# martinResearch/PySparseLP

Hardware: AMD Instinct MI355X
Metric: admm_iterations_per_sec (higher is better)
Workload: dtype f64

## Files before the change

### pysparselp_amd/csrc/slp_tall.h

```cpp
#pragma once
#include "slp_common.h"

namespace slp {

constexpr int kTallC = 4096;
constexpr int kTallT = 1024;
constexpr int kTallSlots = 8;
constexpr int kTallDepth = 4;
constexpr int kTallDictMax = 2048;
constexpr int kTallBuckets = 6;
constexpr int kTallIdBits = 11, kTallColBits = 12, kTallRowBits = 14;
constexpr int kTallCellShift = kTallIdBits + kTallColBits + kTallRowBits;
static_assert(kTallBuckets * 32 == 3 * kWave, "k_tall_build scans the (count, bank class) buckets three per lane of one wave");
static_assert(kTallRmax < (1 << kTallRowBits) && kTallC == (1 << kTallColBits) && kTallDictMax == (1 << kTallIdBits), "tall geometry");
static_assert((kTallRmax + 1) * 8 + kTallDictMax * 8 + 2 * kTallC * 8 <= 160 * 1024, "tall cells: LDS budget");

constexpr unsigned int kPktNewCell = 0x80000000u;
constexpr unsigned int kNoTile = 0x7fffffffu;
constexpr unsigned int kOob = 0xffffff00u;

struct TallPkt {
    unsigned int off;
    unsigned int xsrc;
    unsigned int c[4];
    unsigned int strip;
    unsigned int pad;
};
static_assert(sizeof(TallPkt) == 32, "packet header");

__host__ __device__ inline unsigned long long tall_value_key(unsigned long long bits) {
    return (bits >> 63) ? ~bits : (bits | 0x8000000000000000ull);
}

}
```

### pysparselp_amd/csrc/slp_tall_spmv.hip

```cpp
#include <cmath>
#include <cstdlib>
#include <cstring>
#include <vector>

#include "slp_common.h"
#include "slp_kernels.h"
#include "slp_tall.h"

namespace slp {


template <bool DICT>
struct TallRegs {
    unsigned int lo[kTallSlots];
    unsigned int hi[DICT ? 2 : 1];
    double val[DICT ? 1 : kTallSlots];
    double x[4];
};

template <bool DICT, bool ACC, bool POW = false, int C = kTallC>
__global__ __launch_bounds__(kTallT) void k_tall_spmv(int nseg, const TallWg *__restrict__ wgs, const double *__restrict__ dict_arg,
                                                      const double *__restrict__ x, double *__restrict__ out, double pw) {
    constexpr int kDepth = DICT ? kTallDepth : 2;
    __shared__ double acc[kTallRmax + 1];
    __shared__ double dv[kTallDictMax];
    static_assert(C == 4096 || C == 2048 || C == 1024, "tall cells: strip width");
    __shared__ double xt[2][C];
    constexpr int kPieces = C / 2048 ? C / 2048 : 1;
    const int p = threadIdx.x;
    const bool tile_lane = C >= 2048 || p < C / 2;
    const unsigned int wbase = (unsigned int)__builtin_amdgcn_readfirstlane(p & ~(kWave - 1));
    const int v = blockIdx.x;
    int cur = 0;
    TallWg wg = wgs[v];
    for (int r = p; r <= wg.nrows; r += kTallT) acc[r] = (ACC && r > 0) ? out[wg.row0 + r - 1] : 0.0;
  for (int seg = 0; seg < nseg; ++seg) {
    if (seg > 0) wg = wgs[(i64)seg * gridDim.x + v];
    if (DICT) {
        const double *__restrict__ dsrc = dict_arg ? dict_arg : wg.dict;
        for (int q = p; q < wg.D; q += kTallT) dv[q] = dsrc[q];
    }
    typedef const unsigned int __attribute__((address_space(1))) *gptr_t;
    const gptr_t hd = (gptr_t)(unsigned long long)wg.dir + (p & 7);
    const int npk = (int)wg.npk - 2 * kTallDepth;
    const __amdgpu_buffer_rsrc_t rs_x =
        __builtin_amdgcn_make_buffer_rsrc(const_cast<double *>(x + wg.x0), 0, (int)(wg.ncol * 8), 0x00020000);

    auto slot_pay = [&](unsigned int so, unsigned int width) {
        return __builtin_amdgcn_make_buffer_rsrc(const_cast<unsigned int *>(wg.pay) + so, 0, (int)(width * 4u), 0x00020000);
    };
    auto slot_val = [&](unsigned int so, unsigned int width) {
        return __builtin_amdgcn_make_buffer_rsrc(const_cast<double *>(DICT ? x : wg.val) + so, 0, (int)(width * 8u), 0x00020000);
    };

    TallRegs<DICT> regs[kDepth];
    unsigned int hw[2 * kDepth];

    auto widths = [&](unsigned int h, unsigned int *c) {
#pragma unroll
        for (int i = 0; i < 4; ++i) {
            const unsigned int v = (unsigned int)__builtin_amdgcn_readlane((int)h, 2 + i);
            c[2 * i] = v & 0xffffu;
            c[2 * i + 1] = v >> 16;
        }
    };

    auto load_tile = [&](TallRegs<DICT> &g, const unsigned int xo) {
#pragma unroll
        for (int i = 0; i < kPieces; ++i) {
            const auto v = __builtin_amdgcn_raw_buffer_load_b128(rs_x, xo + (unsigned int)i * (unsigned int)(C * 4), 0, 0);
            g.x[2 * i] = __hiloint2double((int)v[1], (int)v[0]);
            g.x[2 * i + 1] = __hiloint2double((int)v[3], (int)v[2]);
        }
    };

    auto issue = [&](TallRegs<DICT> &g, unsigned int h) {
        const unsigned int off = (unsigned int)__builtin_amdgcn_readlane((int)h, 0);
        const unsigned int xs = (unsigned int)__builtin_amdgcn_readlane((int)h, 1) & 0x7fffffffu;
        unsigned int c[kTallSlots];
        widths(h, c);
        unsigned int so = off;
        const unsigned int mine = (unsigned int)p * 4u;
#pragma unroll
        for (int k = 0; k < kTallSlots; ++k) {
            g.lo[k] = __builtin_amdgcn_raw_buffer_load_b32(slot_pay(so, c[k]), mine, 0, 2);
            if (!DICT) {
                const auto v = __builtin_amdgcn_raw_buffer_load_b64(slot_val(so, c[k]), 2u * mine, 0, 2);
                g.val[k] = __hiloint2double((int)v[1], (int)v[0]);
            }
            so += c[k];
        }
        if (DICT) {
            g.hi[0] = __builtin_amdgcn_raw_buffer_load_b32(slot_pay(so, c[0]), mine, 0, 2);
            so += c[0];
            g.hi[DICT ? 1 : 0] = __builtin_amdgcn_raw_buffer_load_b32(slot_pay(so, c[4]), mine, 0, 2);
        }
        const unsigned int xo = (xs == kNoTile || !tile_lane) ? kOob : (xs + 2u * (unsigned int)p) * 8u;
        load_tile(g, xo);
    };

    auto issue_part = [&](TallRegs<DICT> &g, unsigned int h, const int part) {
        const unsigned int off = (unsigned int)__builtin_amdgcn_readlane((int)h, 0);
        unsigned int c[kTallSlots];
        widths(h, c);
        const unsigned int mine = (unsigned int)p * 4u;
        unsigned int so = off;
        if (part == 1) so += c[0] + c[1] + c[2] + c[3];
        if (part == 0 || wbase < c[4]) {
#pragma unroll
            for (int k = 4 * part; k < 4 * part + 4; ++k) {
                g.lo[k] = __builtin_amdgcn_raw_buffer_load_b32(slot_pay(so, c[k]), mine, 0, 2);
                if (!DICT) {
                    const auto v = __builtin_amdgcn_raw_buffer_load_b64(slot_val(so, c[k]), 2u * mine, 0, 2);
                    g.val[DICT ? 0 : k] = __hiloint2double((int)v[1], (int)v[0]);
                }
                so += c[k];
            }
            if (DICT) {
                if (part == 0) so += c[4] + c[5] + c[6] + c[7];
                else so += c[0];
                g.hi[DICT ? part : 0] = __builtin_amdgcn_raw_buffer_load_b32(slot_pay(so, c[4 * part]), mine, 0, 2);
            }
        }
        if (part == 1) {
            const unsigned int xs = (unsigned int)__builtin_amdgcn_readlane((int)h, 1) & 0x7fffffffu;
            const unsigned int xo = (xs == kNoTile || !tile_lane) ? kOob : (xs + 2u * (unsigned int)p) * 8u;
            load_tile(g, xo);
        }
    };

    auto consume = [&](TallRegs<DICT> &g, unsigned int h, unsigned int hnext, auto &&between) {
        const unsigned int xw = (unsigned int)__builtin_amdgcn_readlane((int)h, 1);
        const unsigned int c4 = (unsigned int)__builtin_amdgcn_readlane((int)h, 4) & 0xffffu;
        if (xw & kPktNewCell) {
            asm volatile("s_waitcnt lgkmcnt(0)\n\ts_barrier" ::: "memory");
            cur ^= 1;
        }
        auto stage_tile = [&]() {
            if ((xw & 0x7fffffffu) != kNoTile) {
                double *dst = &xt[cur ^ 1][2 * p];
                if (tile_lane) *reinterpret_cast<double2 *>(dst) = make_double2(g.x[0], g.x[1]);
                if (kPieces == 2) *reinterpret_cast<double2 *>(dst + C / 2) = make_double2(g.x[2], g.x[3]);
            }
        };
        stage_tile();
        const double *__restrict__ tile = xt[cur];
        auto group = [&](const int k0) {
            unsigned int w[4], hb[4], row[4];
            double ar[4], pr[4], t[4];
#pragma unroll
            for (int k = 0; k < 4; ++k) {
                w[k] = g.lo[k0 + k];
                if (DICT) {
                    hb[k] = (g.hi[DICT ? (k0 >> 2) : 0] >> (8 * k)) & 0xffu;
                    row[k] = (w[k] >> 23) | (hb[k] << 9);
                } else {
                    hb[k] = 0;
                    row[k] = w[k] >> kTallColBits;
                }
            }
#pragma unroll
            for (int k = 0; k < 4; ++k) ar[k] = acc[row[k]];
#pragma unroll
            for (int k = 0; k < 4; ++k) {
                pr[k] = DICT ? dv[w[k] & ((1u << kTallIdBits) - 1)] * tile[(w[k] >> kTallIdBits) & (kTallC - 1)]
                             : (POW ? abs_pow(g.val[DICT ? 0 : k0 + k], pw) * 1.0 : g.val[DICT ? 0 : k0 + k]) * tile[w[k] & (kTallC - 1)];
            }
            t[0] = ar[0] + pr[0];
#pragma unroll
            for (int k = 1; k < 4; ++k) t[k] = ((row[k] == row[k - 1]) ? t[k - 1] : ar[k]) + pr[k];
#pragma unroll
            for (int k = 0; k < 4; ++k) acc[row[k]] = t[k];
        };
        group(0);
        between();
        if (wbase < c4) group(4);
    };

#pragma unroll
    for (int u = 0; u < 2 * kDepth; ++u) hw[u] = hd[(i64)u * 8];
#pragma unroll
    for (int u = 0; u < kDepth; ++u) issue(regs[u], hw[u]);
    __syncthreads();
    for (int jj = 0; jj < npk; jj += 2 * kDepth) {
#pragma unroll
        for (int u = 0; u < 2 * kDepth; ++u) {
            consume(regs[u % kDepth], hw[u], hw[(u + kDepth) % (2 * kDepth)], [&]() { issue_part(regs[u % kDepth], hw[(u + kDepth) % (2 * kDepth)], 0); });
            issue_part(regs[u % kDepth], hw[(u + kDepth) % (2 * kDepth)], 1);
            hw[u] = hd[(i64)(jj + u + 2 * kDepth) * 8];
        }
    }
    __syncthreads();
  }
    for (int r = p; r < wg.nrows; r += kTallT) out[wg.row0 + r] = acc[r + 1];
}


__global__ void k_tall_combine(i64 nrow, int S, const double *__restrict__ part, double *__restrict__ out, int accum) {
    for (i64 r = (i64)blockIdx.x * blockDim.x + threadIdx.x; r < nrow; r += (i64)gridDim.x * blockDim.x) {
        double a = accum ? out[r] + part[r] : part[r];
        for (int s = 1; s < S; ++s) a += part[(i64)s * nrow + r];
        out[r] = a;
    }
}

template <bool DICT, bool ACC, bool POW>
static void tall_launch(int C, unsigned grid, int nseg, const TallWg *wgs, const double *dict, const double *x, double *out, double pw) {
    switch (C) {
    case 4096: hipLaunchKernelGGL((k_tall_spmv<DICT, ACC, POW, 4096>), dim3(grid), dim3(kTallT), 0, ctx().stream, nseg, wgs, dict, x, out, pw); break;
    case 2048: hipLaunchKernelGGL((k_tall_spmv<DICT, ACC, POW, 2048>), dim3(grid), dim3(kTallT), 0, ctx().stream, nseg, wgs, dict, x, out, pw); break;
    case 1024: hipLaunchKernelGGL((k_tall_spmv<DICT, ACC, POW, 1024>), dim3(grid), dim3(kTallT), 0, ctx().stream, nseg, wgs, dict, x, out, pw); break;
    default: SLP_REQUIRE(false, "tall cells: strip width");
    }
}

void tall_spmv(const StripJds &f, const double *x, double *out, int accum) {
    double *dst = f.S > 1 ? f.part.p : out;
    const unsigned grid = (unsigned)(f.B * f.S);
    const bool acc = accum && f.S == 1;
    const double *none = nullptr;
    if (f.D > 0) { if (acc) tall_launch<true, true, false>((int)f.C, grid, 1, f.tall_wg.p, f.dict, x, dst, 0.0); else tall_launch<true, false, false>((int)f.C, grid, 1, f.tall_wg.p, f.dict, x, dst, 0.0); }
    else { if (acc) tall_launch<false, true, false>((int)f.C, grid, 1, f.tall_wg.p, none, x, dst, 0.0); else tall_launch<false, false, false>((int)f.C, grid, 1, f.tall_wg.p, none, x, dst, 0.0); }
    if (f.S > 1)
        hipLaunchKernelGGL(k_tall_combine, dim3(grid_for(f.nrow, kBlock)), dim3(kBlock), 0, ctx().stream, f.nrow, f.S, f.part.p, out, accum);
    SLP_HIP(hipGetLastError());
}

void tall_spmv_fused(const StripJds &f, const double *x, double *out) {
    const int nseg = f.parts_cols ? (int)f.parts.size() : 1;
    const unsigned grid = (unsigned)(f.tall_wg.n / (size_t)nseg);
    if (f.D > 0) tall_launch<true, false, false>((int)f.C, grid, nseg, f.tall_wg.p, nullptr, x, out, 0.0);
    else tall_launch<false, false, false>((int)f.C, grid, nseg, f.tall_wg.p, nullptr, x, out, 0.0);
    SLP_HIP(hipGetLastError());
}

bool tall_fuse(StripJds &f) {
    f.tall_wg.release();
    const char *e = getenv("SLP_TALL_FUSE");
    if (e && e[0] == '0') return false;
    if (f.parts.empty()) return false;
    const StripJds &f0 = *f.parts[0];
    for (const StripJds *g : f.parts)
        if (!g->ok || !g->tall || g->S != 1 || g->C != f0.C || (g->D > 0) != (f0.D > 0) || (f.parts_cols && (g->B != f0.B || g->tall_R != f0.tall_R || g->nrow != f0.nrow)))
            return false;
    std::vector<TallWg> all;
    for (size_t k = 0; k < f.parts.size(); ++k) {
        const StripJds &g = *f.parts[k];
        std::vector<TallWg> wg((size_t)g.B);
        SLP_HIP(hipMemcpy(wg.data(), g.tall_wg.p, wg.size() * sizeof(TallWg), hipMemcpyDeviceToHost));
        for (TallWg &w : wg) {
            w.dict = g.dict;
            if (f.parts_cols) w.x0 = f.part_off[k];
            else w.row0 += f.part_off[k];
            all.push_back(w);
        }
    }
    f.tall_wg.upload(all.data(), all.size());
    f.C = f0.C;
    return true;
}

void tall_spmv_pow(const StripJds &f, double pw, const double *x, double *out, int accum) {
    SLP_REQUIRE(f.ok && f.tall && f.D == 0, "tall_spmv_pow: not a tall-cell copy with fp64 entries");
    double *dst = f.S > 1 ? f.part.p : out;
    const unsigned grid = (unsigned)(f.B * f.S);
    if (accum && f.S == 1) tall_launch<false, true, true>((int)f.C, grid, 1, f.tall_wg.p, nullptr, x, dst, pw);
    else tall_launch<false, false, true>((int)f.C, grid, 1, f.tall_wg.p, nullptr, x, dst, pw);
    if (f.S > 1)
        hipLaunchKernelGGL(k_tall_combine, dim3(grid_for(f.nrow, kBlock)), dim3(kBlock), 0, ctx().stream, f.nrow, f.S, f.part.p, out, accum);
    SLP_HIP(hipGetLastError());
}
}
```

Baseline: 10.69.

## Replace cell-boundary barriers with LDS counter handshakes and rotate wave-to-slot mapping

In the non-POW tall SpMV path, the full workgroup s_barrier at each new cell is replaced by two LDS counters. Waves raise the counters with ds_add and spin-wait on them with s_sleep, which lets waves drift apart instead of all stalling together. Wave lanes now take a packet-specified rotation (lane 6 of the header) to pick which slot range they load. This is meant to balance uneven slot widths across waves. The cost is spin-wait overhead, a trap on timeout, and a new dependency on the packet header format.

```diff
diff --git a/pysparselp_amd/csrc/slp_tall.h b/pysparselp_amd/csrc/slp_tall.h
--- a/pysparselp_amd/csrc/slp_tall.h
+++ b/pysparselp_amd/csrc/slp_tall.h
@@ -7,13 +7,15 @@
 constexpr int kTallT = 1024;
 constexpr int kTallSlots = 8;
 constexpr int kTallDepth = 4;
+constexpr int kTallWaves = kTallT / kWave;
+constexpr unsigned int kTallGiveUp = 1u << 24;
 constexpr int kTallDictMax = 2048;
 constexpr int kTallBuckets = 6;
 constexpr int kTallIdBits = 11, kTallColBits = 12, kTallRowBits = 14;
 constexpr int kTallCellShift = kTallIdBits + kTallColBits + kTallRowBits;
 static_assert(kTallBuckets * 32 == 3 * kWave, "k_tall_build scans the (count, bank class) buckets three per lane of one wave");
 static_assert(kTallRmax < (1 << kTallRowBits) && kTallC == (1 << kTallColBits) && kTallDictMax == (1 << kTallIdBits), "tall geometry");
-static_assert((kTallRmax + 1) * 8 + kTallDictMax * 8 + 2 * kTallC * 8 <= 160 * 1024, "tall cells: LDS budget");
+static_assert((kTallRmax + 1) * 8 + kTallDictMax * 8 + 2 * kTallC * 8 + 2 * 4 <= 160 * 1024, "tall cells: LDS budget");
 
 constexpr unsigned int kPktNewCell = 0x80000000u;
 constexpr unsigned int kNoTile = 0x7fffffffu;
diff --git a/pysparselp_amd/csrc/slp_tall_spmv.hip b/pysparselp_amd/csrc/slp_tall_spmv.hip
--- a/pysparselp_amd/csrc/slp_tall_spmv.hip
+++ b/pysparselp_amd/csrc/slp_tall_spmv.hip
@@ -26,16 +26,24 @@
     __shared__ double dv[kTallDictMax];
     static_assert(C == 4096 || C == 2048 || C == 1024, "tall cells: strip width");
     __shared__ double xt[2][C];
+    __shared__ unsigned int hand[2];
     constexpr int kPieces = C / 2048 ? C / 2048 : 1;
     const int p = threadIdx.x;
     const bool tile_lane = C >= 2048 || p < C / 2;
     const unsigned int wbase = (unsigned int)__builtin_amdgcn_readfirstlane(p & ~(kWave - 1));
+    auto vbase_of = [&](unsigned int h) {
+        if (POW) return wbase;
+        const unsigned int t = (unsigned int)__builtin_amdgcn_readlane((int)h, 6);
+        return (wbase + t * (unsigned int)kWave) & (unsigned int)(kTallT - 1);
+    };
     const int v = blockIdx.x;
     int cur = 0;
     TallWg wg = wgs[v];
     for (int r = p; r <= wg.nrows; r += kTallT) acc[r] = (ACC && r > 0) ? out[wg.row0 + r - 1] : 0.0;
   for (int seg = 0; seg < nseg; ++seg) {
     if (seg > 0) wg = wgs[(i64)seg * gridDim.x + v];
+    if (p < 2) hand[p] = 0u;
+    unsigned int ncell = 0;
     if (DICT) {
         const double *__restrict__ dsrc = dict_arg ? dict_arg : wg.dict;
         for (int q = p; q < wg.D; q += kTallT) dv[q] = dsrc[q];
@@ -80,7 +88,7 @@
         unsigned int c[kTallSlots];
         widths(h, c);
         unsigned int so = off;
-        const unsigned int mine = (unsigned int)p * 4u;
+        const unsigned int mine = (vbase_of(h) + (unsigned int)(p & (kWave - 1))) * 4u;
 #pragma unroll
         for (int k = 0; k < kTallSlots; ++k) {
             g.lo[k] = __builtin_amdgcn_raw_buffer_load_b32(slot_pay(so, c[k]), mine, 0, 2);
@@ -103,10 +111,11 @@
         const unsigned int off = (unsigned int)__builtin_amdgcn_readlane((int)h, 0);
         unsigned int c[kTallSlots];
         widths(h, c);
-        const unsigned int mine = (unsigned int)p * 4u;
+        const unsigned int vbase = vbase_of(h);
+        const unsigned int mine = (vbase + (unsigned int)(p & (kWave - 1))) * 4u;
         unsigned int so = off;
         if (part == 1) so += c[0] + c[1] + c[2] + c[3];
-        if (part == 0 || wbase < c[4]) {
+        if (part == 0 || vbase < c[4]) {
 #pragma unroll
             for (int k = 4 * part; k < 4 * part + 4; ++k) {
                 g.lo[k] = __builtin_amdgcn_raw_buffer_load_b32(slot_pay(so, c[k]), mine, 0, 2);
@@ -129,11 +138,50 @@
         }
     };
 
+    const unsigned int hand_lds = (unsigned int)(size_t)&hand[0];
+    auto wait_for = [&](const int i, const unsigned int target) {
+        unsigned int n, ns, spins;
+        asm volatile("s_mov_b32 %2, 0\n"
+                     "1:\n\t"
+                     "ds_read_b32 %0, %3\n\t"
+                     "s_waitcnt lgkmcnt(0)\n\t"
+                     "v_readfirstlane_b32 %1, %0\n\t"
+                     "s_cmp_ge_u32 %1, %4\n\t"
+                     "s_cbranch_scc1 3f\n\t"
+                     "s_add_u32 %2, %2, 1\n\t"
+                     "s_cmp_eq_u32 %2, %5\n\t"
+                     "s_cbranch_scc0 2f\n\t"
+                     "s_trap 2\n"
+                     "2:\n\t"
+                     "s_sleep 1\n\t"
+                     "s_branch 1b\n"
+                     "3:"
+                     : "=&v"(n), "=&s"(ns), "=&s"(spins)
+                     : "v"(hand_lds + 4u * (unsigned int)i), "s"(target), "i"(kTallGiveUp)
+                     : "memory", "scc");
+    };
+    auto raise = [&](const int i) {
+        unsigned long long saved;
+        asm volatile("s_mov_b64 %0, exec\n\t"
+                     "s_mov_b64 exec, 1\n\t"
+                     "ds_add_u32 %1, %2\n\t"
+                     "s_mov_b64 exec, %0"
+                     : "=&s"(saved)
+                     : "v"(hand_lds + 4u * (unsigned int)i), "v"(1u)
+                     : "memory");
+    };
+
     auto consume = [&](TallRegs<DICT> &g, unsigned int h, unsigned int hnext, auto &&between) {
         const unsigned int xw = (unsigned int)__builtin_amdgcn_readlane((int)h, 1);
         const unsigned int c4 = (unsigned int)__builtin_amdgcn_readlane((int)h, 4) & 0xffffu;
-        if (xw & kPktNewCell) {
+        const bool new_cell = (xw & kPktNewCell) != 0u;
+        if (POW && new_cell) {
             asm volatile("s_waitcnt lgkmcnt(0)\n\ts_barrier" ::: "memory");
+            cur ^= 1;
+        }
+        if (!POW && new_cell) {
+            if (ncell > 0) raise(1);
+            wait_for(0, (unsigned int)kTallWaves * (ncell + 1u));
             cur ^= 1;
         }
         auto stage_tile = [&]() {
@@ -143,11 +191,9 @@
                 if (kPieces == 2) *reinterpret_cast<double2 *>(dst + C / 2) = make_double2(g.x[2], g.x[3]);
             }
         };
-        stage_tile();
         const double *__restrict__ tile = xt[cur];
-        auto group = [&](const int k0) {
-            unsigned int w[4], hb[4], row[4];
-            double ar[4], pr[4], t[4];
+        auto products = [&](const int k0, unsigned int *row, double *pr) {
+            unsigned int w[4], hb[4];
 #pragma unroll
             for (int k = 0; k < 4; ++k) {
                 w[k] = g.lo[k0 + k];
@@ -160,21 +206,39 @@
                 }
             }
 #pragma unroll
-            for (int k = 0; k < 4; ++k) ar[k] = acc[row[k]];
-#pragma unroll
             for (int k = 0; k < 4; ++k) {
                 pr[k] = DICT ? dv[w[k] & ((1u << kTallIdBits) - 1)] * tile[(w[k] >> kTallIdBits) & (kTallC - 1)]
                              : (POW ? abs_pow(g.val[DICT ? 0 : k0 + k], pw) * 1.0 : g.val[DICT ? 0 : k0 + k]) * tile[w[k] & (kTallC - 1)];
             }
+        };
+        auto sums = [&](const unsigned int *row, const double *pr) {
+            double ar[4], t[4];
+#pragma unroll
+            for (int k = 0; k < 4; ++k) ar[k] = acc[row[k]];
             t[0] = ar[0] + pr[0];
 #pragma unroll
             for (int k = 1; k < 4; ++k) t[k] = ((row[k] == row[k - 1]) ? t[k - 1] : ar[k]) + pr[k];
 #pragma unroll
             for (int k = 0; k < 4; ++k) acc[row[k]] = t[k];
         };
-        group(0);
+        unsigned int row[4];
+        double pr[4];
+        if (POW) stage_tile();
+        if (!POW && new_cell) {
+            wait_for(1, (unsigned int)kTallWaves * ncell);
+            ++ncell;
+        }
+        if (!POW && (new_cell || (xw & 0x7fffffffu) != kNoTile)) {
+            stage_tile();
+            raise(0);
+        }
+        products(0, row, pr);
+        sums(row, pr);
         between();
-        if (wbase < c4) group(4);
+        if (vbase_of(h) < c4) {
+            products(4, row, pr);
+            sums(row, pr);
+        }
     };
 
 #pragma unroll
```

New measurement: 9.559, median of 2. -10.6%, worse.
